# Nazukixv/LiteASR

Hardware: AMD Instinct MI355X
Metric: utterances/sec (U2-Conformer+CTC, 80-d fbank T≈1000) at 1/2/4/8 MI355X (higher is better)
Workload: dtype bf16; 1 GPU; U2-Conformer-small hybrid CTC-attention training step (fwd+loss+bwd+allreduce+clip+Noam/Adam); model=U2 enc 12x conformer d256 H4 ff2048, dec 6x, V 4233, global_batch=32, per_gpu_batch=32, seq_len=1000, label_len=40, parallelism=dp1, launch=hipgraph, ranks_seen=1, rank_launcher=env

## Files before the change

### include/liteasr_hip.h

```cpp
#ifndef LITEASR_HIP_H
#define LITEASR_HIP_H

#include <stdint.h>

#ifdef __cplusplus
extern "C" {
#endif

enum { LASR_F32 = 0, LASR_BF16 = 1, LASR_I32 = 2, LASR_I64 = 3, LASR_U8 = 4 };
enum { LASR_OK = 0, LASR_ERR_INVALID = -1, LASR_ERR_LAUNCH = -2 };
enum { LASR_ACT_NONE = 0, LASR_ACT_RELU = 1, LASR_ACT_SWISH = 2,
       LASR_ACT_GATE = 3 ,
       LASR_ACT_TANH = 4  };

const char* lasr_last_error(void);
int lasr_version(void);
int lasr_set_dropout_counter(const uint64_t* dev_counter);
int lasr_counter_add(uint64_t* dev_counter, uint64_t v, void* stream);

typedef struct lasr_gemm_args {
  int M, N, K;
  int batch, batch_div;
  const void* A; int64_t lda_m, lda_k, sa1, sa2;
  const void* B; int64_t ldb_n, ldb_k, sb1, sb2;
  void* C; int64_t ldc, sc1, sc2;
  int in_dtype;
  int c_dtype;
  float alpha; const float* alpha_dev;
  float beta;
  const float* bias;
  int act;
  void* zout;
  const void* aux; int aux_dtype; int64_t ldaux; int aux_act;
  float drop_p; uint64_t drop_seed;
  const void* res; int res_dtype; int64_t ldres; float res_scale;
  int split_k;
  void* workspace; int64_t workspace_bytes;
  float* rowsum;
  int zout_mode;
  int tile_m, tile_n;
  int ksub;
} lasr_gemm_args;
int lasr_gemm(const lasr_gemm_args* args, void* stream);
int lasr_gemm_ln_fwd(const lasr_gemm_args* args, const float* gamma, const float* beta, float eps, void* y,
                     int y_dtype, float* mean, float* rstd, void* stream);
int lasr_gemm_ln_bwd(const lasr_gemm_args* args, const void* x, int x_dtype, const float* gamma, const float* mean,
                     const float* rstd, const void* dres, int dres_dtype, void* dx, int dx_dtype, float* part,
                     int64_t part_floats, void* gb, int gb_dtype, float bscale, float bp, uint64_t bseed,
                     void* stream);
int lasr_gemm_qbias_bwd(const lasr_gemm_args* args, const void* dqu, const void* dqv, int dt, int B, int T, int H,
                        int dk, void* dqkv, int64_t ld, float* ws, int64_t ws_floats, void* stream);
float lasr_dropout_scale(float p);
#define LASR_PLAN_GLDS 1
#define LASR_PLAN_ROWSUM_FUSED 2
#define LASR_PLAN_KSUB2 4
#define LASR_PLAN_WIDE 8
int lasr_gemm_plan(const lasr_gemm_args* args, int* tile_m, int* tile_n, int* split_k, int* flags);

int lasr_gemm_dw_group(const lasr_gemm_args* args, int n, void* stream);
int lasr_gemm_dw_group_order(int longest_first);
int lasr_gemm_narrow_tiles(int on);

typedef struct lasr_reduce_seg {
  const float* part; int64_t N; int P; int accumulate;
  float* out0; float* out1; int64_t split;
} lasr_reduce_seg;
int lasr_reduce_multi(const lasr_reduce_seg* segs, int nseg, void* stream);

int lasr_colsum(const void* X, int dtype, int64_t M, int64_t N, int64_t ldx,
                float* out, int accumulate, float* workspace, int64_t ws_floats, void* stream);

int lasr_layernorm_fwd(const void* x, int x_dtype, int64_t rows, int D, const float* gamma,
                       const float* beta, float eps, void* y, int y_dtype, float* mean,
                       float* rstd, void* y2, int y2_dtype, float p2, uint64_t seed2,
                       void* stream);
int lasr_layernorm2_fwd(const float* x, int64_t rows, int D, const float* g1, const float* b1,
                        const float* g2, const float* b2, float eps, float* y, float* mean1,
                        float* rstd1, void* z, float* mean2, float* rstd2, void* stream);
int lasr_layernorm_bwd(const void* x, int x_dtype, const void* dy, int dy_dtype, int64_t rows,
                       int D, const float* gamma, const float* mean, const float* rstd,
                       const void* dres, int dres_dtype, void* dx, int dx_dtype,
                       float* dgamma, float* dbeta, float* workspace, int64_t ws_floats,
                       void* gb, int gb_dtype, float bscale, float bp, uint64_t bseed,
                       void* stream);
int lasr_layernorm2_bwd(const float* x1, const void* dy1, int dy1_dtype, const float* dres1, int64_t rows, int D,
                        const float* g1, const float* mean1, const float* rstd1, float* part1, const float* x2,
                        const float* g2, const float* mean2, const float* rstd2, float* dx2, float* part2, void* gb2,
                        int gb2_dtype, float bscale, float bp, uint64_t bseed, void* stream);
typedef struct lasr_row_ln_args {
  int M, D, K;
  const void* A; int64_t lda;
  const void* W; int64_t ldw;
  const float* gamma1; const float* beta1; float eps;
  float* mean1; float* rstd1;
  const float* bias; const float* res; float res_scale; float drop_p; uint64_t drop_seed;
  float* out; void* y1; int y1_dtype;
  const float* gamma2; const float* beta2; void* y2; float* mean2; float* rstd2;
  const float* x; const float* dres; float* dx; void* gb; float bscale; float bp; uint64_t bseed;
  float* part; float* dgamma; float* dbeta;
} lasr_row_ln_args;
int lasr_linear_res_ln(const lasr_row_ln_args* args, void* stream);
int lasr_linear_dx_ln_bwd(const lasr_row_ln_args* args, void* stream);

int lasr_branch_grad(const void* dx, int dx_dtype, int64_t n, void* gb, int gb_dtype,
                     float scale, float p, uint64_t seed, void* stream);

int lasr_ctc_fwd(const void* logits, int ldt, int B, int T, int V, int64_t ld, const int32_t* targets,
                 int Lmax, const int32_t* ilen, const int32_t* tlen, float* lse, float* lp,
                 float* alpha, float* beta, float* nll, void* stream);
int lasr_ctc_lattice(int B, int T, int Lmax, const int32_t* targets, const int32_t* ilen, const int32_t* tlen,
                     const float* lp, float* alpha, float* beta, float* nll, void* stream);
int lasr_ctc_bwd(const void* logits, int ldt, int B, int T, int V, int64_t ld, const int32_t* targets,
                 int Lmax, const int32_t* ilen, const int32_t* tlen, const float* lse,
                 const float* lp, const float* alpha, const float* nll, float* beta,
                 int beta_ready, void* grad, int gdt, float gscale, const float* gdev, void* stream);

int lasr_lsm_kl_fwd(const void* logits, int ldt, int R, int V, int64_t ld, const int32_t* target,
                    int ignore, float smoothing, float* lse, float* loss_rows, void* stream);
int lasr_lsm_kl_bwd(const void* logits, int ldt, int R, int V, int64_t ld, const int32_t* target,
                    int ignore, float smoothing, const float* lse, void* grad, int gdt,
                    float gscale, const float* gdev, void* stream);
int lasr_loss_combine(const float* a, int na, float wa, const float* b, int nb, float wb,
                      float* out, void* stream);

int lasr_qbias_fwd(const void* qkv, int dt, int B, int T, int H, int dk, int64_t ld_qkv,
                   const float* bias_u, const float* bias_v, void* qu, void* qv, void* stream);
int lasr_qbias_bwd(const void* dqu, const void* dqv, int dt, int B, int T, int H, int dk,
                   void* dqkv, int64_t ld_dqkv, float* dbias_u, float* dbias_v,
                   float* workspace, int64_t ws_floats, void* stream);
int lasr_attn_softmax_fwd(const float* s_ac, const float* s_bd, int relpos, int B, int H,
                          int Tq, int Tk, int ldS, const uint8_t* mask, int64_t mask_sb,
                          int64_t mask_sq, void* P, int pdt, float drop_p, uint64_t seed,
                          void* Praw, void* stream);
int lasr_attn_softmax_bwd(const void* P, int pdt, const float* dPd, int B, int H, int Tq, int Tk,
                          int ldS, const uint8_t* mask, int64_t mask_sb, int64_t mask_sq,
                          float drop_p, uint64_t seed, void* dS, int dsdt, void* stream);
int lasr_relshift_bwd(const void* dS, int dt, int Z, int T, int ldS, void* dBD, void* stream);
int lasr_relattn_fwd(const void* qu, const void* qv, int64_t ldq, const void* k, const void* v,
                     int64_t ldkv, const void* pos, int64_t ldp, int B, int H, int T, int dk,
                     const uint8_t* mask, int64_t mask_sb, int64_t mask_sq, float scale,
                     float* stats, void* ctx, int64_t ldc, void* stream);
int lasr_relattn_fwd_qb(const void* q, int64_t ldqin, const float* bu, const float* bv, void* qu, void* qv,
                        int64_t ldq, const void* k, const void* v, int64_t ldkv, const void* pos, int64_t ldp,
                        int B, int H, int T, int dk, const uint8_t* mask, int64_t mask_sb, int64_t mask_sq,
                        float scale, float* stats, void* ctx, int64_t ldc, void* stream);
int lasr_relattn_bwd(const void* qu, const void* qv, int64_t ldq, const void* k, const void* v,
                     int64_t ldkv, const void* pos, int64_t ldp, int B, int H, int T, int dk,
                     const uint8_t* mask, int64_t mask_sb, int64_t mask_sq, float scale,
                     const float* stats, const void* ctx, const void* dctx, int64_t ldc,
                     float* Dbuf, void* dqu, void* dbd, int ldS, int dbd_head_major, void* dk_out,
                     void* dv_out, int64_t lddkv, void* stream);
int lasr_attn_fwd(const void* q, int64_t ldq, const void* k, const void* v, int64_t ldkv, int B, int H,
                  int Tq, int Tk, int dk, const uint8_t* mask, int64_t mask_sb, int64_t mask_sq, float scale,
                  float* stats, void* ctx, int64_t ldc, void* stream);
int lasr_attn_bwd(const void* q, int64_t ldq, const void* k, const void* v, int64_t ldkv, int B, int H,
                  int Tq, int Tk, int dk, const uint8_t* mask, int64_t mask_sb, int64_t mask_sq, float scale,
                  const float* stats, const void* ctx, const void* dctx, int64_t ldc, float* Dbuf, void* dq,
                  void* dk_out, void* dv_out, int64_t lddkv, void* stream);
int lasr_attn_fwd_split(const void* q, int64_t ldq, const void* k, const void* v, int64_t ldkv, int B, int H,
                        int Tq, int Tk, int dk, const uint8_t* mask, int64_t mask_sb, int64_t mask_sq, float scale,
                        float* stats, void* ctx, int64_t ldc, int nsplit, float* work, int64_t work_floats,
                        void* stream);
int lasr_attn_bwd_split(const void* q, int64_t ldq, const void* k, const void* v, int64_t ldkv, int B, int H,
                        int Tq, int Tk, int dk, const uint8_t* mask, int64_t mask_sb, int64_t mask_sq, float scale,
                        const float* stats, const void* ctx, const void* dctx, int64_t ldc, float* Dbuf, void* dq,
                        void* dk_out, void* dv_out, int64_t lddkv, int nsplit, float* work, int64_t work_floats,
                        void* stream);
int64_t lasr_attn_split_work(int B, int H, int Tq, int dk, int nsplit);
int lasr_attn_split_count(int B, int H, int Tq, int Tk);
int lasr_reduce_batch(const float* src, int B, int H, int T, int dk, void* dst, int dt,
                      void* stream);

int lasr_conv1_fwd(const float* x, int B, int T, int F, int C, const float* w,
                   const float* bias, void* y1, int dt, void* stream);
int lasr_conv1_bwd(const float* x, int B, int T, int F, int C, const void* dy1, int dt,
                   float* dw, float* db, float* workspace, int64_t ws_floats, void* stream);
int lasr_im2col3x3s2(const void* y1, int dt, int B, int T1, int F1, int C, void* col,
                     void* stream);
int lasr_col2im3x3s2(const void* dcol, int dt, int B, int T1, int F1, int C,
                     const void* y1, void* dy1, void* stream);
#define LASR_CONV2_FWD 0
#define LASR_CONV2_DW 1
#define LASR_CONV2_DX 2
#define LASR_CONV2_DX_W1 3
typedef struct lasr_conv2_args {
  int mode;
  int B, T1, F1, C;
  const void* y1;
  const void* w2p;
  const float* bias;
  const void* dy2; int64_t dy2_rows;
  void* out;
  float* rowsum;
  void* workspace; int64_t workspace_bytes;
  const float* x; int T, F;
  float* dw1; float* db1;
} lasr_conv2_args;
int lasr_conv2_gemm(const lasr_conv2_args* args, void* stream);
int64_t lasr_conv2_dx_w1_workspace(int B, int T1, int F1, int C);
typedef struct lasr_cif_args {
  int B, T, D, U;
  const float* z; const int* plen; const int* ylen; const float* h;
  float* alpha; float* acc; uint8_t* fired; int* row; float* sum_alpha; float* mae; float* out;
  const float* gout; const float* gsum; float* dz; float* dh;
} lasr_cif_args;
int lasr_cif_fwd(const lasr_cif_args* args, void* stream);
int lasr_cif_bwd(const lasr_cif_args* args, void* stream);
typedef struct lasr_cif_infer_args {
  int B, T, D;
  const float* z; const int* plen; const float* h;
  float* alpha; float* acc; uint8_t* fired; int* row; float* sum_alpha; int* ulen; int* count; float* out;
} lasr_cif_infer_args;
int lasr_cif_infer(const lasr_cif_infer_args* args, void* stream);
int lasr_glancing_mix(int64_t rows, int D, const uint8_t* replace, const float* a, const float* b,
// ... 171 lines not shown
```

### liteasr_amd/_native.py

```python

from __future__ import annotations

import ctypes as C
import os

_HERE = os.path.dirname(os.path.abspath(__file__))
LIB_PATH = os.path.join(_HERE, "lib", "libliteasr_hip.so")

F32, BF16, I32, I64, U8 = 0, 1, 2, 3, 4
ACT_NONE, ACT_RELU, ACT_SWISH, ACT_GATE, ACT_TANH = 0, 1, 2, 3, 4

_p = C.c_void_p
_i = C.c_int
_l = C.c_int64
_f = C.c_float
_u = C.c_uint64


class GemmArgs(C.Structure):

    _fields_ = [
        ("M", _i), ("N", _i), ("K", _i),
        ("batch", _i), ("batch_div", _i),
        ("A", _p), ("lda_m", _l), ("lda_k", _l), ("sa1", _l), ("sa2", _l),
        ("B", _p), ("ldb_n", _l), ("ldb_k", _l), ("sb1", _l), ("sb2", _l),
        ("C", _p), ("ldc", _l), ("sc1", _l), ("sc2", _l),
        ("in_dtype", _i), ("c_dtype", _i),
        ("alpha", _f), ("alpha_dev", _p),
        ("beta", _f),
        ("bias", _p),
        ("act", _i),
        ("zout", _p),
        ("aux", _p), ("aux_dtype", _i), ("ldaux", _l), ("aux_act", _i),
        ("drop_p", _f), ("drop_seed", _u),
        ("res", _p), ("res_dtype", _i), ("ldres", _l), ("res_scale", _f),
        ("split_k", _i), ("workspace", _p), ("workspace_bytes", _l),
        ("rowsum", _p),
        ("zout_mode", _i),
        ("tile_m", _i), ("tile_n", _i), ("ksub", _i),
    ]


class Conv2Args(C.Structure):

    _fields_ = [
        ("mode", _i),
        ("B", _i), ("T1", _i), ("F1", _i), ("C", _i),
        ("y1", _p), ("w2p", _p), ("bias", _p),
        ("dy2", _p), ("dy2_rows", _l),
        ("out", _p), ("rowsum", _p),
        ("workspace", _p), ("workspace_bytes", _l),
        ("x", _p), ("T", _i), ("F", _i),
        ("dw1", _p), ("db1", _p),
    ]


CONV2_FWD, CONV2_DW, CONV2_DX, CONV2_DX_W1 = 0, 1, 2, 3


class CifArgs(C.Structure):

    _fields_ = [
        ("B", _i), ("T", _i), ("D", _i), ("U", _i),
        ("z", _p), ("plen", _p), ("ylen", _p), ("h", _p),
        ("alpha", _p), ("acc", _p), ("fired", _p), ("row", _p), ("sum_alpha", _p), ("mae", _p), ("out", _p),
        ("gout", _p), ("gsum", _p), ("dz", _p), ("dh", _p),
    ]


class CifInferArgs(C.Structure):

    _fields_ = [
        ("B", _i), ("T", _i), ("D", _i),
        ("z", _p), ("plen", _p), ("h", _p),
        ("alpha", _p), ("acc", _p), ("fired", _p), ("row", _p), ("sum_alpha", _p), ("ulen", _p), ("count", _p),
        ("out", _p),
    ]


class RowLnArgs(C.Structure):

    _fields_ = [
        ("M", _i), ("D", _i), ("K", _i),
        ("A", _p), ("lda", _l), ("W", _p), ("ldw", _l),
        ("gamma1", _p), ("beta1", _p), ("eps", _f), ("mean1", _p), ("rstd1", _p),
        ("bias", _p), ("res", _p), ("res_scale", _f), ("drop_p", _f), ("drop_seed", _u),
        ("out", _p), ("y1", _p), ("y1_dtype", _i),
        ("gamma2", _p), ("beta2", _p), ("y2", _p), ("mean2", _p), ("rstd2", _p),
        ("x", _p), ("dres", _p), ("dx", _p), ("gb", _p), ("bscale", _f), ("bp", _f), ("bseed", _u),
        ("part", _p), ("dgamma", _p), ("dbeta", _p),
    ]


class ReduceSeg(C.Structure):

    _fields_ = [("part", _p), ("N", _l), ("P", _i), ("accumulate", _i), ("out0", _p), ("out1", _p),
                ("split", _l)]


RNNT_SEARCH_MAX_LAYERS = 8


class RnntSearchArgs(C.Structure):

    _fields_ = [
        ("Tcap", _i), ("layers", _i), ("dec_dim", _i), ("H", _i), ("J", _i), ("V", _i),
        ("node_cap", _i), ("slot_cap", _i),
        ("w_dtype", _i),
        ("arena", _p), ("arena_bytes", _l),
        ("embed", _p),
        ("Wih", _p * RNNT_SEARCH_MAX_LAYERS), ("Whh", _p * RNNT_SEARCH_MAX_LAYERS),
        ("bih", _p * RNNT_SEARCH_MAX_LAYERS), ("bhh", _p * RNNT_SEARCH_MAX_LAYERS),
        ("Wd", _p), ("Wj", _p), ("bj", _p), ("enc_proj", _p),
    ]


SIGNATURES = {
    "lasr_version": [],
    "lasr_last_error": [],
    "lasr_set_dropout_counter": [_p],
    "lasr_counter_add": [_p, _u, _p],
    "lasr_gemm": [C.POINTER(GemmArgs), _p],
    "lasr_gemm_plan": [C.POINTER(GemmArgs), _p, _p, _p, _p],
    "lasr_gemm_dw_group": [C.POINTER(GemmArgs), _i, _p],
    "lasr_gemm_dw_group_order": [_i],
    "lasr_gemm_narrow_tiles": [_i],
    "lasr_relattn_fwd": [_p, _p, _l, _p, _p, _l, _p, _l, _i, _i, _i, _i, _p, _l, _l, _f, _p, _p, _l, _p],
    "lasr_relattn_fwd_qb": [_p, _l, _p, _p, _p, _p, _l, _p, _p, _l, _p, _l, _i, _i, _i, _i, _p, _l, _l, _f, _p, _p,
                            _l, _p],
    "lasr_attn_fwd": [_p, _l, _p, _p, _l, _i, _i, _i, _i, _i, _p, _l, _l, _f, _p, _p, _l, _p],
    "lasr_attn_bwd": [_p, _l, _p, _p, _l, _i, _i, _i, _i, _i, _p, _l, _l, _f, _p, _p, _p, _l, _p, _p, _p, _p,
                      _l, _p],
    "lasr_attn_fwd_split": [_p, _l, _p, _p, _l, _i, _i, _i, _i, _i, _p, _l, _l, _f, _p, _p, _l, _i, _p, _l, _p],
    "lasr_attn_bwd_split": [_p, _l, _p, _p, _l, _i, _i, _i, _i, _i, _p, _l, _l, _f, _p, _p, _p, _l, _p, _p, _p,
                            _p, _l, _i, _p, _l, _p],
    "lasr_attn_split_work": [_i, _i, _i, _i, _i],
    "lasr_attn_split_count": [_i, _i, _i, _i],
    "lasr_relattn_bwd": [_p, _p, _l, _p, _p, _l, _p, _l, _i, _i, _i, _i, _p, _l, _l, _f, _p, _p, _p, _l,
                         _p, _p, _p, _i, _i, _p, _p, _l, _p],
    "lasr_reduce_multi": [C.POINTER(ReduceSeg), _i, _p],
    "lasr_linear_res_ln": [C.POINTER(RowLnArgs), _p],
    "lasr_linear_dx_ln_bwd": [C.POINTER(RowLnArgs), _p],
    "lasr_dropout_scale": [_f],
    "lasr_colsum": [_p, _i, _l, _l, _l, _p, _i, _p, _l, _p],
    "lasr_layernorm2_fwd": [_p, _l, _i, _p, _p, _p, _p, _f, _p, _p, _p, _p, _p, _p, _p],
    "lasr_layernorm_fwd": [_p, _i, _l, _i, _p, _p, _f, _p, _i, _p, _p, _p, _i, _f, _u, _p],
    "lasr_layernorm_bwd": [_p, _i, _p, _i, _l, _i, _p, _p, _p, _p, _i, _p, _i, _p, _p, _p, _l,
                           _p, _i, _f, _f, _u, _p],
    "lasr_layernorm2_bwd": [_p, _p, _i, _p, _l, _i, _p, _p, _p, _p, _p, _p, _p, _p, _p, _p, _p, _i, _f, _f, _u,
                            _p],
    "lasr_branch_grad": [_p, _i, _l, _p, _i, _f, _f, _u, _p],
    "lasr_ctc_fwd": [_p, _i, _i, _i, _i, _l, _p, _i, _p, _p, _p, _p, _p, _p, _p, _p],
    "lasr_ctc_lattice": [_i, _i, _i, _p, _p, _p, _p, _p, _p, _p, _p],
    "lasr_rnnt_fwd": [_p, _i, _i, _i, _i, _i, _l, _p, _i, _p, _p, _i, _p, _p, _p, _p, _p, _p],
    "lasr_rnnt_bwd": [_p, _i, _i, _i, _i, _i, _l, _p, _i, _p, _p, _i, _p, _p, _p, _p, _p, _p, _i, _f, _p, _p],
    "lasr_joint_fwd": [_p, _p, _i, _i, _i, _i, _p, _i, _p],
    "lasr_joint_reduce": [_p, _i, _i, _i, _i, _i, _p, _p, _i, _p],
    "lasr_lstm_cell_fwd": [_p, _l, _p, _p, _i, _i, _p, _p, _i, _l, _p],
    "lasr_lstm_cell_bwd": [_p, _l, _p, _p, _p, _p, _i, _l, _p, _p, _i, _i, _p, _i, _l, _p, _p],
    "lasr_ctc_bwd": [_p, _i, _i, _i, _i, _l, _p, _i, _p, _p, _p, _p, _p, _p, _p, _i, _p, _i, _f, _p, _p],
    "lasr_lsm_kl_fwd": [_p, _i, _i, _i, _l, _p, _i, _f, _p, _p, _p],
    "lasr_lsm_kl_bwd": [_p, _i, _i, _i, _l, _p, _i, _f, _p, _p, _i, _f, _p, _p],
    "lasr_loss_combine": [_p, _i, _f, _p, _i, _f, _p, _p],
    "lasr_qbias_fwd": [_p, _i, _i, _i, _i, _i, _l, _p, _p, _p, _p, _p],
    "lasr_qbias_bwd": [_p, _p, _i, _i, _i, _i, _i, _p, _l, _p, _p, _p, _l, _p],
    "lasr_attn_softmax_fwd": [_p, _p, _i, _i, _i, _i, _i, _i, _p, _l, _l, _p, _i, _f, _u, _p, _p],
    "lasr_attn_softmax_bwd": [_p, _i, _p, _i, _i, _i, _i, _i, _p, _l, _l, _f, _u, _p, _i, _p],
    "lasr_relshift_bwd": [_p, _i, _i, _i, _i, _p, _p],
    "lasr_reduce_batch": [_p, _i, _i, _i, _i, _p, _i, _p],
    "lasr_conv1_fwd": [_p, _i, _i, _i, _i, _p, _p, _p, _i, _p],
    "lasr_conv1_bwd": [_p, _i, _i, _i, _i, _p, _i, _p, _p, _p, _l, _p],
    "lasr_conv2_gemm": [C.POINTER(Conv2Args), _p],
    "lasr_conv2_dx_w1_workspace": [_i, _i, _i, _i],
    "lasr_cif_fwd": [C.POINTER(CifArgs), _p],
    "lasr_cif_bwd": [C.POINTER(CifArgs), _p],
    "lasr_cif_infer": [C.POINTER(CifInferArgs), _p],
    "lasr_glancing_mix": [_l, _i, _p, _p, _p, _p, _p, _i, _p],
    "lasr_im2col3x3s2": [_p, _i, _i, _i, _i, _i, _p, _p],
    "lasr_col2im3x3s2": [_p, _i, _i, _i, _i, _i, _p, _p, _p],
    "lasr_permute_last2": [_p, _i, _l, _l, _l, _p, _i, _i, _i, _p],
    "lasr_glu_dwconv_fwd": [_p, _i, _i, _i, _i, _i, _p, _p, _p, _i, _p, _p],
    "lasr_dwconv_nparts": [_i, _i],
    "lasr_bn_finalize": [_p, _i, _i, _f, _f, _p, _p, _p, _p, _p, _p, _p, _p, _p, _i, _p],
    "lasr_bn_act_fwd": [_p, _i, _l, _i, _p, _p, _p, _i, _i, _p],
    "lasr_bn_act_bwd": [_p, _i, _p, _i, _l, _i, _p, _p, _p, _p, _p, _p, _p, _p, _i, _p, _l, _i, _i, _p],
    "lasr_glu_dwconv_bwd": [_p, _i, _p, _i, _i, _i, _i, _i, _p, _p, _p, _p, _p, _l, _p],
    "lasr_bn_act_glu_dwconv_bwd": [_p, _i, _p, _i, _i, _i, _i, _p, _p, _p, _p, _p, _p, _p, _p, _l, _i, _i,
                                   _p, _i, _i, _p, _p, _p, _p, _p, _l, _p],
    "lasr_cast": [_p, _i, _p, _i, _l, _p],
    "lasr_scale_add": [_p, _i, _p, _i, _f, _f, _p, _i, _l, _p],
    "lasr_embed_pe_fwd": [_p, _i, _i, _i, _p, _p, _f, _f, _u, _p, _i, _p],
    "lasr_embed_bwd": [_p, _i, _i, _p, _i, _f, _f, _u, _p, _p],
    "lasr_pe_fwd": [_p, _i, _l, _i, _i, _p, _f, _f, _u, _p, _i, _p],
    "lasr_u2_prep": [_p, _p, _p, _i, _i, _i, _i, _i, _i, _i, _p, _p, _p, _p, _p, _p, _p, _p],
    "lasr_u2_prep_ld": [_p, _p, _p, _i, _i, _i, _i, _i, _i, _i, _p, _p, _p, _p, _i, _p, _i, _p, _p, _p],
    "lasr_gemm_qbias_bwd": [C.POINTER(GemmArgs), _p, _p, _i, _i, _i, _i, _i, _p, _l, _p, _l, _p],
    "lasr_gemm_ln_fwd": [C.POINTER(GemmArgs), _p, _p, _f, _p, _i, _p, _p, _p],
    "lasr_gemm_ln_bwd": [C.POINTER(GemmArgs), _p, _i, _p, _p, _p, _p, _i, _p, _i, _p, _l, _p, _i, _f, _f, _u, _p],
    "lasr_u2_prep_chunk": [_p, _p, _p, _i, _i, _i, _i, _i, _i, _i, _p, _p, _u, _i,
                           _p, _p, _p, _p, _i, _p, _p, _i, _p, _p, _p],
    "lasr_pcm_to_float": [_p, _l, _p, _p],
    "lasr_fbank": [_p, _l, _i, _l, _p, _i, _p, _p, _i, _p, _p, _p, _i, _p],
    "lasr_resample_i16": [_p, _l, _i, _l, _p, _p, _i, _p, _l, _p, _l, _l, _p],
    "lasr_sumsq_nparts": [_l],
    "lasr_sumsq_partial": [_p, _l, _p, _l, _p],
    "lasr_adam_step": [_p, _p, _i, _p, _p, _p, _l, _p, _i, _p, _f, _i, _f, _f, _f, _f, _f, _f,
                       _f, _f, _p],
    "lasr_fill": [_p, _i, _l, _f, _p],
    "lasr_spec_augment": [_p, _p, _p, _p, _i, _i, _i, _i, _i, _p, _l, _p],
    "lasr_spec_augment_ws_bytes": [_i, _i],
    "lasr_logsoftmax_topk": [_p, _i, _l, _i, _l, _i, _p, _p, _p, _p, _p],
    "lasr_rnnt_search_workspace": [_i, _i, _i, _i, _i, _i, _i],
    "lasr_rnnt_search_init": [C.POINTER(RnntSearchArgs), _i, _p],
    "lasr_rnnt_search_expand": [C.POINTER(RnntSearchArgs), _i, _p],
    "lasr_rescore_workspace": [_i, _i],
    "lasr_rescore_search": [_p, _l, _i, _i, _i, _i, _i, _p, _p, _p, _p],
    "lasr_rescore_prep": [_p, _l, _i, _i, _i, _i, _p, _p, _i, _p, _p, _p],
    "lasr_rescore_pick": [_p, _l, _i, _i, _p, C.c_double, _p],
    "lasr_w2v_conv0_fwd": [_p, _i, _i, _i, _i, _i, _p, _p, _p, _p],
    "lasr_w2v_conv0_dw_parts": [_i, _i],
    "lasr_w2v_conv0_dw": [_p, _p, _i, _i, _i, _i, _i, _i, _p, _p, _l, _p],
    "lasr_w2v_ln_act_fwd": [_p, _i, _l, _i, _p, _p, _f, _i, _p, _i, _p, _p, _p],
    "lasr_w2v_ln_act_bwd": [_p, _i, _p, _i, _l, _i, _p, _p, _p, _p, _i, _p, _i, _p, _p, _p, _l, _p],
    "lasr_w2v_col2im1d": [_p, _i, _i, _i, _i, _i, _i, _i, _p, _p],
    "lasr_w2v_group_pack": [_p, _i, _i, _i, _i, _i, _i, _p, _i, _p, _p, _i, _p],
    "lasr_w2v_group_unpack": [_p, _i, _p, _i, _p, _i, _i, _i, _i, _p, _p],
    "lasr_w2v_group_colsum": [_p, _i, _i, _l, _i, _p, _p],
    "lasr_w2v_mask_fwd": [_p, _p, _i, _i, _i, _i, _p, _p],
    "lasr_w2v_mask_bwd": [_p, _p, _i, _i, _i, _i, _p, _p],
    "lasr_w2v_gather_rows": [_p, _i, _l, _l, _p, _i, _i, _i, _i, _p, _i, _p],
    "lasr_w2v_scatter_rows": [_p, _i, _p, _i, _i, _i, _i, _p, _l, _l, _i, _p],
    "lasr_w2v_gumbel_fwd": [_p, _i, _p, _u, _f, _i, _l, _i, _i, _p, _i, _p, _i, _p, _p],
    "lasr_w2v_gumbel_bwd": [_p, _i, _p, _u, _f, _i, _l, _i, _i, _p, _i, _p, _i, _p, _p, _i, _p, _p],
    "lasr_w2v_contrast_fwd": [_p, _p, _p, _p, _i, _i, _i, _i, _i, _f, _p, _p, _p, _p, _p],
    "lasr_w2v_contrast_bwd": [_p, _p, _p, _p, _i, _i, _i, _i, _i, _f, _p, _p, _p, _p, _p, _l, _p],
}
_RESTYPES = {"lasr_last_error": C.c_char_p, "lasr_spec_augment_ws_bytes": C.c_int64,
             "lasr_rnnt_search_workspace": C.c_int64, "lasr_rescore_workspace": C.c_int64,
             "lasr_conv2_dx_w1_workspace": C.c_int64, "lasr_attn_split_work": C.c_int64,
             "lasr_dropout_scale": C.c_float}


class NativeError(RuntimeError):
    pass


_lib = None


def load():
    global _lib
    if _lib is not None:
        return _lib
    want = os.environ.get("LITEASR_HIP_LIB")
    if want and os.path.abspath(want) != os.path.abspath(LIB_PATH):
        raise NativeError(f"LITEASR_HIP_LIB={want} does not select the library (this process loads {LIB_PATH}); "
                          "run `python tools/with_lib.py LIB script.py` to use another build")
    if not os.path.exists(LIB_PATH):
        raise NativeError(
            f"libliteasr_hip.so not found at {LIB_PATH}; build it with `make` "
            "(the HIP path has no fallback)"
        )
    lib = C.CDLL(LIB_PATH)
    for name, argtypes in SIGNATURES.items():
        fn = getattr(lib, name)
        fn.argtypes = argtypes
        fn.restype = _RESTYPES.get(name, C.c_int)
    _lib = lib
    return lib


def call(name, *args):
    lib = _lib if _lib is not None else load()
    rc = getattr(lib, name)(*args)
    if rc != 0:
        msg = lib.lasr_last_error().decode(errors="replace")
        raise NativeError(f"{name} failed ({rc}): {msg}")
    return rc


def exported_symbols():
    return sorted(SIGNATURES)
```

### liteasr_amd/csrc/gemm.hip

```cpp
#include "gemm_kernel.h"
#include <algorithm>


template <bool AKC, bool BKC, typename TC>
void launch_bf16(const GemmP& p, int BM, int BN, int ks, int nw, bool glds, dim3 grid, hipStream_t st);
#define LASR_EXTERN_LAUNCH(ak, bk)                                                                         \
  extern template void launch_bf16<ak, bk, float>(const GemmP&, int, int, int, int, bool, dim3, hipStream_t); \
  extern template void launch_bf16<ak, bk, bf16_t>(const GemmP&, int, int, int, int, bool, dim3, hipStream_t);
LASR_EXTERN_LAUNCH(true, true)
LASR_EXTERN_LAUNCH(true, false)
LASR_EXTERN_LAUNCH(false, true)
LASR_EXTERN_LAUNCH(false, false)
#undef LASR_EXTERN_LAUNCH

template <typename TC>
static void dispatch(const GemmP& p, bool akc, bool bkc, int bf16in, int BM, int BN, int ks, int nw, bool glds,
                     dim3 grid, hipStream_t st) {
  if (bf16in) {
    if (akc && bkc) launch_bf16<true, true, TC>(p, BM, BN, ks, nw, glds, grid, st);
    else if (akc) launch_bf16<true, false, TC>(p, BM, BN, ks, nw, glds, grid, st);
    else if (bkc) launch_bf16<false, true, TC>(p, BM, BN, ks, nw, glds, grid, st);
    else launch_bf16<false, false, TC>(p, BM, BN, ks, nw, glds, grid, st);
  } else {
    if (akc && bkc) gemm_f32_kernel<true, true, TC><<<grid, 256, 0, st>>>(p);
    else if (akc) gemm_f32_kernel<true, false, TC><<<grid, 256, 0, st>>>(p);
    else if (bkc) gemm_f32_kernel<false, true, TC><<<grid, 256, 0, st>>>(p);
    else gemm_f32_kernel<false, false, TC><<<grid, 256, 0, st>>>(p);
  }
}

static int narrow_n_tiles = 1;
extern "C" int lasr_gemm_narrow_tiles(int on) {
  narrow_n_tiles = on != 0;
  return LASR_OK;
}

static void gemm_plan(const lasr_gemm_args* a, int* BMo, int* BNo, int* splito, int* kso = nullptr,
                      int* nwo = nullptr) {
  int nw = 4;
  const int batch = a->batch > 0 ? a->batch : 1;
  const bool bf = a->in_dtype == LASR_BF16;
  int BM = 64, BN = 64;
  int split = a->split_k > 0 ? a->split_k : 1;
  const bool plain = !a->act && !a->zout && !a->aux && !a->res && a->drop_p <= 0.f;
  const bool autosplit = a->split_k <= 0 && !a->zout && a->workspace;
  const int kt = (int)cdiv(a->K, 32);
  if (bf && autosplit && kt >= 16) {
    const bool very_long = kt >= 2048;
    BM = BN = 64;
    if (very_long) {
      BM = a->M >= 96 ? 128 : 64;
      BN = a->N >= 96 ? 128 : 64;
    } else if ((int64_t)a->M * a->N > 768 * 256) {
      BM = a->M >= a->N ? 64 : 128;
      BN = a->M >= a->N ? 128 : 64;
    }
    const int64_t nb = cdiv(a->M, BM) * cdiv(a->N, BN) * (int64_t)batch;
    const int64_t target = a->lda_k == 1 ? 128 : (very_long || !plain ? 256 : 512);
    while (nb * split < target && split * 2 <= 64 && kt / (split * 2) >= 8) split *= 2;
  } else if (bf) {
    const int cfg[4][2] = {{128, 128}, {128, 64}, {64, 128}, {64, 64}};
    const int c0 = a->N <= 64 && narrow_n_tiles ? 3 : 0;
    for (int c = c0; c < 4; ++c) {
      const int64_t nb = cdiv(a->M, cfg[c][0]) * cdiv(a->N, cfg[c][1]) * (int64_t)batch;
      BM = cfg[c][0]; BN = cfg[c][1];
      if (nb >= 480) break;
    }
    if (BM == 128 && BN == 128 && a->N >= 256 && a->K >= 1024 && cdiv(a->M, 128) * batch >= 1024) BN = 256;
    if (BM == 128 && BN == 128 && (a->zout || a->aux || (a->act && a->drop_p > 0.f)) && a->N >= 1024) BN = 256;
  }
  if (!bf && autosplit) {
    const int64_t nb = cdiv(a->M, BM) * cdiv(a->N, BN) * (int64_t)batch;
    while (nb * split < 512 && split * 2 <= 32 && kt / (split * 2) >= 4) split *= 2;
  }
  if (bf && a->tile_m) {
    BM = a->tile_m;
    BN = a->tile_n;
    nw = 4;
  }
  if (a->split_k <= -2 && plain && a->workspace) split = -a->split_k;
  const int64_t rs_floats = a->rowsum ? (int64_t)split * a->M : 0;
  if (split > 1 && ((!plain && !autosplit && (a->split_k < 2 || a->zout)) || !a->workspace ||
                    a->workspace_bytes < ((int64_t)split * batch * a->M * a->N + rs_floats) * 4))
    split = 1;
  if (kso) {
    const int64_t kc = split > 1 ? cdiv(a->K, split) : a->K;
    const bool small = BM * BN <= 64 * 128;
    *kso = (bf && BM < 256 && BN < 256 && ((BM == 64 && BN == 64) || kc >= 1024 || (kc >= 512 && small))) ? 2 : 1;
    if (nw == 8) *kso = 2;
    else if (a->ksub) *kso = a->ksub;
  }
  if (nwo) *nwo = nw;
  *BMo = BM;
  *BNo = BN;
  *splito = split;
}

static bool gemm_uses_glds(const lasr_gemm_args* a) {
  if (a->in_dtype != LASR_BF16) return false;
  const bool akc = (a->lda_k == 1), bkc = (a->ldb_k == 1);
  const int64_t s_a = akc ? a->lda_m : a->lda_k;
  const int64_t s_b = bkc ? a->ldb_n : a->ldb_k;
  const bool a_vec = aligned16(a->A) && s_a % 8 == 0 && a->sa1 % 8 == 0 && a->sa2 % 8 == 0;
  const bool b_vec = aligned16(a->B) && s_b % 8 == 0 && a->sb1 % 8 == 0 && a->sb2 % 8 == 0;
  const int64_t M8 = cdiv(a->M, 8) * 8, N8 = cdiv(a->N, 8) * 8;
  return a_vec && b_vec && (akc || a->lda_k >= M8) && (bkc || a->ldb_k >= N8);
}

static bool tile_ok(int tm, int tn) {
  return (tm == 0 && tn == 0) || ((tm == 64 || tm == 128 || tm == 256) && (tn == 64 || tn == 128 || tn == 256) &&
                                  (tm < 256 || tn >= 128) && (tn < 256 || tm >= 128));
}

extern "C" int lasr_gemm_plan(const lasr_gemm_args* a, int* tile_m, int* tile_n, int* split_k, int* flags) {
  LASR_CHECK_ARG(a && tile_m && tile_n && split_k, "lasr_gemm_plan: null argument");
  int ks = 1, nw = 4;
  gemm_plan(a, tile_m, tile_n, split_k, &ks, &nw);
  const bool glds = gemm_uses_glds(a);
  if (!glds) {
    *tile_m = std::min(*tile_m, 128);
    *tile_n = std::min(*tile_n, 128);
    nw = 4;
  }
  if (flags) {
    *flags = (glds ? LASR_PLAN_GLDS : 0) | (a->rowsum && glds && a->lda_k != 1 ? LASR_PLAN_ROWSUM_FUSED : 0) |
             (glds && ks == 2 && (*tile_m < 256 || nw == 8) ? LASR_PLAN_KSUB2 : 0) |
             (glds && nw == 8 ? LASR_PLAN_WIDE : 0);
  }
  return LASR_OK;
}

extern "C" int lasr_gemm(const lasr_gemm_args* a, void* stream) { return gemm_run(a, stream, nullptr); }

int gemm_run(const lasr_gemm_args* a, void* stream, GemmRowPost* post) {
  LASR_CHECK_ARG(a != nullptr, "lasr_gemm: null args");
  LASR_CHECK_ARG(a->M >= 0 && a->N >= 0 && a->K >= 0, "lasr_gemm: negative size");
  LASR_CHECK_ARG(a->in_dtype == LASR_F32 || a->in_dtype == LASR_BF16, "lasr_gemm: bad in_dtype");
  LASR_CHECK_ARG(a->c_dtype == LASR_F32 || a->c_dtype == LASR_BF16, "lasr_gemm: bad c_dtype");
  LASR_CHECK_ARG(a->lda_m == 1 || a->lda_k == 1, "lasr_gemm: A needs a unit stride");
  LASR_CHECK_ARG(a->ldb_n == 1 || a->ldb_k == 1, "lasr_gemm: B needs a unit stride");
  LASR_CHECK_ARG(a->A && a->B && a->C, "lasr_gemm: null operand");
  LASR_CHECK_ARG(a->zout_mode == 0 || a->zout_mode == 1, "lasr_gemm: zout_mode must be 0 or 1");
  LASR_CHECK_ARG(a->act != LASR_ACT_GATE && (!a->aux || a->aux_act != LASR_ACT_NONE),
                 "lasr_gemm: act GATE is only an aux_act; aux needs an aux_act");
  LASR_CHECK_ARG(tile_ok(a->tile_m, a->tile_n) && a->ksub >= 0 && a->ksub <= 2,
                 "lasr_gemm: tile override must be 64/128/256 x 64/128/256 (256 only beside >= 128) or 0 x 0, "
                 "ksub 0, 1 or 2");
  if (a->M == 0 || a->N == 0 || a->batch == 0) return LASR_OK;
  const int batch = a->batch > 0 ? a->batch : 1;
  const int bdiv = a->batch_div > 0 ? a->batch_div : 1;
  LASR_CHECK_ARG(batch == 1 || (!a->aux && !a->res && !a->zout && !a->rowsum),
                 "lasr_gemm: aux/res/zout/rowsum only supported for batch == 1");
  LASR_CHECK_ARG(!a->rowsum || a->lda_m == 1, "lasr_gemm: rowsum needs an M-contiguous A");

  GemmP p;
  p.M = a->M; p.N = a->N; p.K = a->K; p.batch = batch; p.batch_div = bdiv;
  p.A = a->A; p.lda_m = a->lda_m; p.lda_k = a->lda_k; p.sa1 = a->sa1; p.sa2 = a->sa2;
  p.B = a->B; p.ldb_n = a->ldb_n; p.ldb_k = a->ldb_k; p.sb1 = a->sb1; p.sb2 = a->sb2;
  p.C = a->C; p.ldc = a->ldc; p.sc1 = a->sc1; p.sc2 = a->sc2;
  p.alpha = a->alpha; p.alpha_dev = a->alpha_dev; p.beta = a->beta;
  p.bias = a->bias; p.act = a->act; p.zout = a->zout; p.zout_mode = a->zout_mode;
  p.aux = a->aux; p.aux_dtype = a->aux_dtype; p.ldaux = a->ldaux; p.aux_act = a->aux_act;
  p.drop = mkdrop(a->drop_p, a->drop_seed);
  p.res = a->res; p.res_dtype = a->res_dtype; p.ldres = a->ldres; p.res_scale = a->res_scale;

  const bool akc = (a->lda_k == 1);
  const bool bkc = (a->ldb_k == 1);
  const bool bf = a->in_dtype == LASR_BF16;
  {
    const int64_t s_a = akc ? a->lda_m : a->lda_k;
    const int64_t s_b = bkc ? a->ldb_n : a->ldb_k;
    p.a_vec = bf && aligned16(a->A) && s_a % 8 == 0 && a->sa1 % 8 == 0 && a->sa2 % 8 == 0;
    p.b_vec = bf && aligned16(a->B) && s_b % 8 == 0 && a->sb1 % 8 == 0 && a->sb2 % 8 == 0;
  }
  p.c_vec = aligned16(a->C) && a->ldc % 8 == 0 && a->sc1 % 8 == 0 && a->sc2 % 8 == 0 &&
            (!a->zout || aligned16(a->zout));
  p.aux_vec = a->aux && aligned16(a->aux) && a->ldaux % 8 == 0;
  p.res_vec = a->res && aligned16(a->res) && a->ldres % 8 == 0;
  p.ws_vec = a->N % 8 == 0;
  p.bias_vec = a->bias && aligned16(a->bias);
  {
    auto al4 = [](const void* q, int dtp) {
      return ((uintptr_t)q & (dtp == LASR_F32 ? 15 : 7)) == 0;
    };
    const int cdt = a->c_dtype;
    p.v4 = a->N % 4 == 0 && a->ldc % 4 == 0 && a->sc1 % 4 == 0 && a->sc2 % 4 == 0 && al4(a->C, cdt) &&
           (!a->zout || al4(a->zout, cdt)) && (!a->bias || aligned16(a->bias)) &&
           (!a->aux || (a->ldaux % 4 == 0 && al4(a->aux, a->aux_dtype))) &&
           (!a->res || (a->ldres % 4 == 0 && al4(a->res, a->res_dtype))) &&
           (!a->workspace || aligned16(a->workspace));
  }
  {
    const int nsrc = (a->aux ? 1 : 0) + (a->res ? 1 : 0);
    const bool base_ok = p.c_vec && a->beta == 0.f;
    const bool src_ok = nsrc == 1 && a->N % 8 == 0 && (a->aux ? p.aux_vec : p.res_vec);
    p.epi_mode = !base_ok ? 2 : nsrc == 0 ? 0 : src_ok ? 1 : 2;
  }

  int BM, BN, split, ks, nw;
  gemm_plan(a, &BM, &BN, &split, &ks, &nw);
  p.split_k = split;
  const int kstep = bf ? 32 : 16;
  p.kchunk = split > 1 ? (int)(cdiv(cdiv(a->K, split), kstep) * kstep) : a->K;
  p.ws = (float*)a->workspace;
  p.rowsum = nullptr;
  p.rs_ws = nullptr;

  hipStream_t st = (hipStream_t)stream;
  const bool glds = gemm_uses_glds(a);
  if (!glds) {
    BM = std::min(BM, 128);
    BN = std::min(BN, 128);
    nw = 4;
  }
  dim3 grid((unsigned)cdiv(a->N, BN), (unsigned)cdiv(a->M, BM), (unsigned)(batch * split));
  LASR_CHECK_ARG(grid.y <= 65535 && grid.z <= 65535, "lasr_gemm: grid too large");
  const bool rs_fused = a->rowsum && glds && !akc;
  if (rs_fused) {
    p.rowsum = a->rowsum;
    if (split > 1) p.rs_ws = p.ws + (int64_t)split * batch * a->M * a->N;
  }
  if (a->c_dtype == LASR_F32) dispatch<float>(p, akc, bkc, bf, BM, BN, ks, nw, glds, grid, st);
  else dispatch<bf16_t>(p, akc, bkc, bf, BM, BN, ks, nw, glds, grid, st);
  int rc = lasr_check_launch("lasr_gemm");
  if (!rc && split > 1 && a->split_k >= 0 && post) {
    const int r = post->launch(p, post->ctx, st);
    if (r < 0) return r;
    post->done = r;
    if (r) {
      rc = lasr_check_launch("lasr_gemm/splitk_reduce_post");
      if (rc || !a->rowsum || rs_fused) return rc;
    }
  }
  if (!rc && split > 1 && a->split_k >= 0 && !(post && post->done)) {
    const int64_t total = (int64_t)a->M * a->N * batch;
    const int nblk = (int)std::min<int64_t>(cdiv(p.v4 ? total / 4 : total, 256), 4096);
    if (a->c_dtype == LASR_F32) splitk_reduce_kernel<float><<<nblk, 256, 0, st>>>(p);
    else splitk_reduce_kernel<bf16_t><<<nblk, 256, 0, st>>>(p);
    rc = lasr_check_launch("lasr_gemm/splitk_reduce");
  }
  if (rc || !a->rowsum || rs_fused) return rc;
  const int64_t used = split > 1 ? (int64_t)split * batch * a->M * a->N : 0;
  LASR_CHECK_ARG(a->workspace && a->workspace_bytes / 4 > used, "lasr_gemm: no workspace left for the rowsum");
  return lasr_colsum(a->A, a->in_dtype, a->K, a->M, a->lda_k, a->rowsum, 1, (float*)a->workspace + used,
                     a->workspace_bytes / 4 - used, stream);
}


int launch_dw_group(const DwGroupP& g, int BM, int BN, int blocks, bool serial, hipStream_t st);
static int dw_group_lpt = 1;
extern "C" int lasr_gemm_dw_group_order(int longest_first) {
  dw_group_lpt = longest_first != 0;
  return LASR_OK;
}

extern "C" int lasr_gemm_dw_group(const lasr_gemm_args* args, int n, void* stream) {
  LASR_CHECK_ARG(args && n >= 1 && n <= LASR_DW_GROUP_MAX, "lasr_gemm_dw_group: 1..%d problems", LASR_DW_GROUP_MAX);
  DwGroupP g = {};
  g.n = n;
  int ord[LASR_DW_GROUP_MAX];
  int64_t work[LASR_DW_GROUP_MAX];
  auto planned = [](const lasr_gemm_args* a) {
    lasr_gemm_args b = *a;
    if (b.split_k <= -2 && !b.workspace) {
      b.workspace = (void*)(uintptr_t)16;
      b.workspace_bytes = INT64_MAX;
    }
    return b;
  };
  for (int i = 0; i < n; ++i) {
    const lasr_gemm_args pa = planned(args + i), *a = &pa;
    int bm, bn, sp, ks;
    gemm_plan(a, &bm, &bn, &sp, &ks);
    work[i] = a->split_k == 1 || sp <= 1 ? a->K : cdiv(a->K, sp);
    ord[i] = i;
  }
  if (dw_group_lpt && !(args[0].split_k <= -2 && !args[0].workspace))
    std::stable_sort(ord, ord + n, [&](int x, int y) { return work[x] > work[y]; });
  int BM0 = 0, BN0 = 0, blocks = 0;
  bool all_serial = false;
  for (int i = 0; i < n; ++i) {
    const bool serial = args[ord[i]].split_k <= -2 && !args[ord[i]].workspace;
    const lasr_gemm_args pa = planned(args + ord[i]), *a = &pa;
    LASR_CHECK_ARG(a->in_dtype == LASR_BF16 && a->c_dtype == LASR_F32, "lasr_gemm_dw_group: bf16 in, fp32 partials");
    LASR_CHECK_ARG(a->lda_m == 1 && a->lda_k != 1 && a->ldb_n == 1 && a->ldb_k != 1,
                   "lasr_gemm_dw_group: A M-contiguous and B N-contiguous (dW = dY^T X)");
    const bool direct = a->split_k == 1;
    LASR_CHECK_ARG((direct || (a->split_k < 0 && a->workspace)) && (a->batch <= 1) && a->M > 0 && a->N > 0 &&
                       a->K > 0,
                   "lasr_gemm_dw_group: partials-only problems with a workspace, or direct (split_k 1) ones");
    LASR_CHECK_ARG(!serial || (a->C && a->ldc >= a->N && (a->beta == 0.f || a->beta == 1.f) && a->alpha == 1.f &&
                               !a->alpha_dev && a->split_k >= -64),
                   "lasr_gemm_dw_group: a serial problem needs C, ldc >= N, beta 0 or 1, alpha 1, <= 64 slices");
    LASR_CHECK_ARG(i == 0 || serial == all_serial, "lasr_gemm_dw_group: serial and slab problems mixed");
    all_serial = serial;
    LASR_CHECK_ARG(!direct || (a->C && a->ldc >= a->N && (a->beta == 0.f || a->beta == 1.f) && a->alpha == 1.f &&
                               !a->alpha_dev),
                   "lasr_gemm_dw_group: a direct problem needs C, ldc >= N, beta 0 or 1, alpha 1");
    LASR_CHECK_ARG(i == 0 || direct == (g.direct[0] != 0), "lasr_gemm_dw_group: direct and split problems mixed");
    LASR_CHECK_ARG(!a->act && !a->zout && !a->aux && !a->res && a->drop_p <= 0.f && !a->bias,
                   "lasr_gemm_dw_group: no epilogue");
    LASR_CHECK_ARG(gemm_uses_glds(a), "lasr_gemm_dw_group: operands not LDS-DMA eligible");
    int BM, BN, split, ks;
    gemm_plan(a, &BM, &BN, &split, &ks);
    if (direct) split = 2;
    LASR_CHECK_ARG(split > 1, "lasr_gemm_dw_group: plan is not a split-K launch");
    if (((BM == 128 && BN == 64) || (BM == 64 && BN == 128)) && a->M >= 128 && a->N >= 128) {
      BM = BN = 128;
      if (a->M >= 256 && a->N >= 256 && !direct) {
        BM = 256;
        BN = 128;
      }
    }
    LASR_CHECK_ARG(i == 0 || (BM == BM0 && BN == BN0), "lasr_gemm_dw_group: problems plan different tiles");
    BM0 = BM;
    BN0 = BN;
    if (direct) split = 1;
    g.M[i] = a->M; g.N[i] = a->N; g.K[i] = a->K;
    g.split[i] = split;
    g.kchunk[i] = direct ? a->K : (int)(cdiv(cdiv(a->K, split), 32) * 32);
    g.direct[i] = direct;
    g.C[i] = (float*)a->C; g.ldc[i] = a->ldc; g.beta[i] = a->beta; g.rowsum[i] = a->rowsum;
    g.v4[i] = serial ? a->N % 4 == 0 && aligned16(a->C) && a->ldc % 4 == 0
                     : a->N % 4 == 0 && aligned16(direct ? a->C : a->workspace);
    g.A[i] = a->A; g.lda[i] = a->lda_k;
    g.B[i] = a->B; g.ldb[i] = a->ldb_k;
    g.ws[i] = serial ? nullptr : (float*)a->workspace;
    g.rs_ws[i] = a->rowsum && !direct && !serial ? (float*)a->workspace + (int64_t)split * a->M * a->N : nullptr;
    g.start[i] = blocks;
    const int64_t nb = cdiv(a->M, BM) * cdiv(a->N, BN) * (int64_t)(serial ? 1 : split);
    LASR_CHECK_ARG(blocks + nb + 8 < (1ll << 31), "lasr_gemm_dw_group: too many blocks");
    blocks += (int)cdiv(nb, 8) * 8;
  }
  g.start[n] = blocks;
  static const int slice_xcd = [] { const char* e = getenv("LASR_DW_SLICE_XCD"); return e && e[0] ? atoi(e) : 1; }();
  g.slice_xcd = slice_xcd;
  LASR_CHECK_ARG(launch_dw_group(g, BM0, BN0, blocks, all_serial, (hipStream_t)stream) == 0,
                 "lasr_gemm_dw_group: no grouped instance for tile %dx%d", BM0, BN0);
  return lasr_check_launch("lasr_gemm_dw_group");
}
```

Measured before the change: 3514 utterances/sec.

## Add phased software-pipelined GEMM kernel for single-wave large-K shapes

Adds a specialized 128x64 bf16 GEMM kernel with a 6-stage global-to-LDS ring buffer. It interleaves MFMA issue with LDS fragment reads and DMA issue under scheduling barriers and raised wave priority. The path is used by default (mode 1) only for GEMMs with K>=1024 whose tile count falls between 3/4 and 1x the CU count, with plain bf16 or residual-dropout f32 epilogues. The aim is to hide memory latency on occupancy-1, single-wave GEMMs such as the FF2048 down-projection. It adds a launch counter and a mode switch. The risk is lower throughput than the existing tuned kernels on the shapes it takes over.

```diff
diff --git a/include/liteasr_hip.h b/include/liteasr_hip.h
--- a/include/liteasr_hip.h
+++ b/include/liteasr_hip.h
@@ -60,6 +60,8 @@
 int lasr_gemm_dw_group(const lasr_gemm_args* args, int n, void* stream);
 int lasr_gemm_dw_group_order(int longest_first);
 int lasr_gemm_narrow_tiles(int on);
+int lasr_gemm_phased(int mode);
+long long lasr_gemm_phased_launches(void);
 
 typedef struct lasr_reduce_seg {
   const float* part; int64_t N; int P; int accumulate;
diff --git a/liteasr_amd/_native.py b/liteasr_amd/_native.py
--- a/liteasr_amd/_native.py
+++ b/liteasr_amd/_native.py
@@ -125,6 +125,8 @@
     "lasr_gemm_dw_group": [C.POINTER(GemmArgs), _i, _p],
     "lasr_gemm_dw_group_order": [_i],
     "lasr_gemm_narrow_tiles": [_i],
+    "lasr_gemm_phased": [_i],
+    "lasr_gemm_phased_launches": [],
     "lasr_relattn_fwd": [_p, _p, _l, _p, _p, _l, _p, _l, _i, _i, _i, _i, _p, _l, _l, _f, _p, _p, _l, _p],
     "lasr_relattn_fwd_qb": [_p, _l, _p, _p, _p, _p, _l, _p, _p, _l, _p, _l, _i, _i, _i, _i, _p, _l, _l, _f, _p, _p,
                             _l, _p],
@@ -238,7 +240,7 @@
 _RESTYPES = {"lasr_last_error": C.c_char_p, "lasr_spec_augment_ws_bytes": C.c_int64,
              "lasr_rnnt_search_workspace": C.c_int64, "lasr_rescore_workspace": C.c_int64,
              "lasr_conv2_dx_w1_workspace": C.c_int64, "lasr_attn_split_work": C.c_int64,
-             "lasr_dropout_scale": C.c_float}
+             "lasr_dropout_scale": C.c_float, "lasr_gemm_phased_launches": C.c_int64}
 
 
 class NativeError(RuntimeError):
diff --git a/liteasr_amd/csrc/gemm.hip b/liteasr_amd/csrc/gemm.hip
--- a/liteasr_amd/csrc/gemm.hip
+++ b/liteasr_amd/csrc/gemm.hip
@@ -1,4 +1,5 @@
 #include "gemm_kernel.h"
+#include "gemm_phase.h"
 #include <algorithm>
 
 
@@ -220,9 +221,12 @@
     p.rowsum = a->rowsum;
     if (split > 1) p.rs_ws = p.ws + (int64_t)split * batch * a->M * a->N;
   }
-  if (a->c_dtype == LASR_F32) dispatch<float>(p, akc, bkc, bf, BM, BN, ks, nw, glds, grid, st);
+  const bool phased = gemm_phased_launch(a, p, glds, st);
+  if (phased) {
+  } else if (a->c_dtype == LASR_F32) dispatch<float>(p, akc, bkc, bf, BM, BN, ks, nw, glds, grid, st);
   else dispatch<bf16_t>(p, akc, bkc, bf, BM, BN, ks, nw, glds, grid, st);
   int rc = lasr_check_launch("lasr_gemm");
+  if (phased && !rc) gemm_phased_count();
   if (!rc && split > 1 && a->split_k >= 0 && post) {
     const int r = post->launch(p, post->ctx, st);
     if (r < 0) return r;
diff --git a/liteasr_amd/csrc/gemm_phase.h b/liteasr_amd/csrc/gemm_phase.h
--- /dev/null
+++ b/liteasr_amd/csrc/gemm_phase.h
@@ -0,0 +1,5 @@
+#pragma once
+#include "gemm_kernel.h"
+
+bool gemm_phased_launch(const lasr_gemm_args* a, const GemmP& p, bool glds, hipStream_t st);
+void gemm_phased_count();
diff --git a/liteasr_amd/csrc/gemm_phase.hip b/liteasr_amd/csrc/gemm_phase.hip
--- /dev/null
+++ b/liteasr_amd/csrc/gemm_phase.hip
@@ -0,0 +1,255 @@
+#include "gemm_phase.h"
+
+#include <atomic>
+#include <type_traits>
+
+namespace {
+
+constexpr int PH_BM = 128, PH_BN = 64;
+
+template <int GL, int NMAX>
+LASR_DEV void wait_stages(int n) {
+  if constexpr (NMAX > 0) {
+    if (n >= NMAX) { wait_vmcnt<GL * NMAX>(); return; }
+    wait_stages<GL, NMAX - 1>(n);
+  } else {
+    wait_vmcnt<0>();
+  }
+}
+
+LASR_DEV v4i ds_b128_at(uint32_t addr, int off) {
+  v4i r;
+  asm volatile("ds_read_b128 %0, %1 offset:%2" : "=v"(r) : "v"(addr), "n"(off));
+  return r;
+}
+LASR_DEV v2i ds_tr_at(uint32_t addr) {
+  v2i r;
+  asm volatile("ds_read_b64_tr_b16 %0, %1" : "=v"(r) : "v"(addr));
+  return r;
+}
+
+template <bool BKC>
+struct PhaseFrags {
+  v4i a[4];
+  v4i bk[BKC ? 2 : 1];
+  v2i bt[BKC ? 1 : 4];
+};
+
+template <bool BKC>
+LASR_DEV void frags_wait(PhaseFrags<BKC>& f) {
+  if constexpr (BKC)
+    asm volatile("s_waitcnt lgkmcnt(0)"
+                 : "+v"(f.a[0]), "+v"(f.a[1]), "+v"(f.a[2]), "+v"(f.a[3]), "+v"(f.bk[0]), "+v"(f.bk[1]));
+  else
+    asm volatile("s_waitcnt lgkmcnt(0)"
+                 : "+v"(f.a[0]), "+v"(f.a[1]), "+v"(f.a[2]), "+v"(f.a[3]), "+v"(f.bt[0]), "+v"(f.bt[1]),
+                   "+v"(f.bt[2]), "+v"(f.bt[3]));
+}
+
+LASR_DEV void pin() { __builtin_amdgcn_sched_barrier(0); }
+
+template <bool BKC, typename TC, int EPI, int S>
+__global__ __launch_bounds__(256, 1) void gemm_phase_kernel(GemmP p) {
+  constexpr int BM = PH_BM, BN = PH_BN, BK = 32, NT = 256;
+  constexpr int WM = 64, WN = 32, FM = 4, FN = 2;
+  constexpr int TILE = (BM + BN) * BK;
+  constexpr int STAGE = 2 * TILE, D = S - 1, GL = 2 * (BM + BN) * 4 / NT;
+  constexpr int MAIN_BYTES = S * STAGE * 2, EPI_BYTES = WM * (BN + 4) * 4;
+  static_assert(S >= 5, "vmcnt(GL * (D - 3)) must leave a stage in flight");
+  static_assert(MAIN_BYTES >= EPI_BYTES && MAIN_BYTES <= 160 * 1024, "ring size");
+  static_assert(GL * (D - 3) < 64, "vmcnt range");
+  __shared__ __attribute__((aligned(16))) char smem_epi[MAIN_BYTES];
+  bf16_t* smem = reinterpret_cast<bf16_t*>(smem_epi);
+  const int tid = threadIdx.x, lane = tid & 63, wid = tid >> 6;
+  const int wr = wid >> 1, wc = wid & 1;
+
+  const int nx = gridDim.x, ny = gridDim.y;
+  const int wg = xcd_remap(blockIdx.y * nx + blockIdx.x, nx * ny);
+  const int tx = wg % nx, ty = wg / nx;
+  const int m0 = ty * BM, n0 = tx * BN;
+  const int nst = p.K / (2 * BK);
+
+  f32x4 acc[FM][FN];
+#pragma unroll
+  for (int i = 0; i < FM; ++i)
+#pragma unroll
+    for (int j = 0; j < FN; ++j) acc[i][j] = (f32x4){0.f, 0.f, 0.f, 0.f};
+
+  uint32_t va[2], vb;
+#pragma unroll
+  for (int i = 0; i < 2; ++i) {
+    const int P = i * NT + tid, r = P >> 2, c = (P & 3) ^ swz(r);
+    va[i] = 2u * ((uint32_t)min(m0 + r, p.M - 1) * (uint32_t)p.lda_m + (uint32_t)c * 8u);
+  }
+  if constexpr (BKC) {
+    const int r = tid >> 2, c = (tid & 3) ^ swz(r);
+    vb = 2u * ((uint32_t)min(n0 + r, p.N - 1) * (uint32_t)p.ldb_n + (uint32_t)c * 8u);
+  } else {
+    constexpr int CPR = BN / 8;
+    const int k = tid / CPR, ps = tid % CPR;
+    const int ls = ((((ps >> 1) ^ htr<BN>(k))) << 1) | (ps & 1);
+    const int gc = min(n0 + ls * 8, ((p.N + 7) & ~7) - 8);
+    vb = 2u * ((uint32_t)k * (uint32_t)p.ldb_k + (uint32_t)gc);
+  }
+  const char* adma = (const char*)p.A;
+  const char* bdma = (const char*)p.B;
+  const int64_t bstep = BKC ? 2 * BK : 2 * BK * p.ldb_k;
+  const int wid_s = __builtin_amdgcn_readfirstlane(wid);
+  auto issue_sub = [&](int slot, int u) {
+    if (LASR_EXP & 4) return;
+    bf16_t* dst = smem + slot * STAGE + u * TILE + wid_s * 512;
+    __builtin_amdgcn_global_load_lds((gptr_t)(adma + va[0]), (lptr_t)dst, 16, 0, 0);
+    __builtin_amdgcn_global_load_lds((gptr_t)(adma + va[1]), (lptr_t)(dst + NT * 8), 16, 0, 0);
+    __builtin_amdgcn_global_load_lds((gptr_t)(bdma + vb), (lptr_t)(dst + BM * BK), 16, 0, 0);
+  };
+  auto advance = [&]() {
+    adma += 2 * BK;
+    bdma += bstep;
+  };
+
+  const uint32_t lds0 = (uint32_t)(uintptr_t)(lptr_t)smem;
+  const uint32_t a_off = lds0 + 2u * (uint32_t)lds_off(wr * WM + (lane & 15), lane >> 4);
+  [[maybe_unused]] const uint32_t bk_off =
+      lds0 + 2u * (uint32_t)(BM * BK + lds_off(wc * WN + (lane & 15), lane >> 4));
+  [[maybe_unused]] uint32_t bt_off[FN][2];
+  if constexpr (!BKC)
+#pragma unroll
+    for (int j = 0; j < FN; ++j) {
+      frag_tr_offsets<BN>(wc * WN + j * 16, lane, bt_off[j]);
+      bt_off[j][0] += lds0 + 2u * BM * BK;
+      bt_off[j][1] += lds0 + 2u * BM * BK;
+    }
+  auto read_part = [&](PhaseFrags<BKC>& f, uint32_t sub, int n) {
+    if (n == 0) {
+      f.a[0] = ds_b128_at(a_off + sub, 0);
+      f.a[1] = ds_b128_at(a_off + sub, 1024);
+    } else if (n == 1) {
+      f.a[2] = ds_b128_at(a_off + sub, 2048);
+      f.a[3] = ds_b128_at(a_off + sub, 3072);
+    } else if constexpr (BKC) {
+      f.bk[0] = ds_b128_at(bk_off + sub, 0);
+      f.bk[1] = ds_b128_at(bk_off + sub, 1024);
+    } else {
+      f.bt[0] = ds_tr_at(bt_off[0][0] + sub);
+      f.bt[1] = ds_tr_at(bt_off[0][1] + sub);
+      f.bt[2] = ds_tr_at(bt_off[1][0] + sub);
+      f.bt[3] = ds_tr_at(bt_off[1][1] + sub);
+    }
+  };
+  auto mfma = [&](const PhaseFrags<BKC>& f, int n) {
+    const int i = n >> 1, j = n & 1;
+    const bf16x8 af = __builtin_bit_cast(bf16x8, f.a[i]);
+    bf16x8 bfr;
+    if constexpr (BKC) bfr = __builtin_bit_cast(bf16x8, f.bk[j]);
+    else bfr = frag_from_raw(f.bt + 2 * j);
+    if (LASR_EXP & 1) {
+      acc[i][j][0] += (float)af[0] + (float)bfr[0];
+      return;
+    }
+    acc[i][j] = __builtin_amdgcn_mfma_f32_16x16x32_bf16(bfr, af, acc[i][j], 0, 0, 0);
+  };
+  auto group = [&](const PhaseFrags<BKC>& cur, PhaseFrags<BKC>& nxt, uint32_t nsub, bool dma, int slot, int u) {
+    __builtin_amdgcn_s_setprio(1);
+#pragma unroll
+    for (int n = 0; n < 8; ++n) {
+      mfma(cur, n);
+      pin();
+      if (n < 3) read_part(nxt, nsub, n);
+      pin();
+    }
+    if (dma) issue_sub(slot, u);
+    advance();
+    pin();
+    __builtin_amdgcn_s_setprio(0);
+  };
+
+  PhaseFrags<BKC> f0, f1;
+#pragma unroll
+  for (int t = 0; t < D; ++t)
+    if (t < nst) {
+      issue_sub(t, 0);
+      advance();
+      issue_sub(t, 1);
+      advance();
+    }
+  wait_stages<GL, D - 2>(min(D, nst) - 2);
+  __builtin_amdgcn_s_barrier();
+#pragma unroll
+  for (int n = 0; n < 3; ++n) read_part(f0, 0u, n);
+  int slot = 0;
+  for (int kt = 0; kt < nst; ++kt) {
+    const bool dma = kt + D < nst;
+    if (kt + D <= nst) wait_vmcnt<GL * (D - 3)>();
+    else wait_stages<GL, D - 3>(nst - 1 - (kt + 2));
+    __builtin_amdgcn_s_barrier();
+    const int nslot = slot + 1 == S ? 0 : slot + 1;
+    const int dslot = slot == 0 ? S - 1 : slot - 1;
+    const uint32_t sub0 = (uint32_t)slot * (STAGE * 2);
+    frags_wait<BKC>(f0);
+    group(f0, f1, sub0 + TILE * 2, dma, dslot, 0);
+    frags_wait<BKC>(f1);
+    group(f1, f0, (uint32_t)nslot * (STAGE * 2), dma, dslot, 1);
+    slot = nslot;
+  }
+  asm volatile("s_waitcnt lgkmcnt(0)" ::: "memory");
+  __syncthreads();
+  __builtin_assume(p.split_k <= 1 && p.epi_mode < 2);
+  gemm_epilogue<BM, BN, TC, true, G_LIN, 4, EPI>(p, acc, smem_epi, m0, n0, 0, 0, 0, 0);
+}
+
+constexpr int PH_S = 6;
+
+template <bool BKC>
+void launch_phase(const GemmP& p, int epi, dim3 grid, hipStream_t st) {
+  if (epi == EPI_RES_DROP) gemm_phase_kernel<BKC, float, EPI_RES_DROP, PH_S><<<grid, 256, 0, st>>>(p);
+  else gemm_phase_kernel<BKC, bf16_t, EPI_PLAIN, PH_S><<<grid, 256, 0, st>>>(p);
+}
+
+std::atomic<long long> phased_launches{0};
+std::atomic<int> phased_mode{1};
+
+int cu_count() {
+  static const int n = [] {
+    int dev = 0, v = 0;
+    if (hipGetDevice(&dev) != hipSuccess) return 0;
+    if (hipDeviceGetAttribute(&v, hipDeviceAttributeMultiprocessorCount, dev) != hipSuccess) return 0;
+    return v;
+  }();
+  return n;
+}
+
+}
+
+bool gemm_phased_launch(const lasr_gemm_args* a, const GemmP& p, bool glds, hipStream_t st) {
+  const int mode = phased_mode.load(std::memory_order_relaxed);
+  if (!mode) return false;
+  if (!glds || a->lda_k != 1 || p.batch != 1 || p.split_k > 1 || a->rowsum || a->zout) return false;
+  if (a->K < 64 || a->K % 64 != 0) return false;
+  const int e = epi_code(p);
+  const bool res_drop = e == EPI_RES_DROP && a->c_dtype == LASR_F32;
+  const bool plain = e == EPI_PLAIN && a->c_dtype == LASR_BF16;
+  if (!res_drop && !plain) return false;
+  const bool bkc = a->ldb_k == 1;
+  const int64_t a_bytes = 2 * (int64_t)a->M * a->lda_m, b_bytes = 2 * (bkc ? (int64_t)a->N * a->ldb_n : 32 * a->ldb_k);
+  if (a_bytes >= (1ll << 32) || b_bytes >= (1ll << 32)) return false;
+  const int64_t tiles = cdiv(a->M, PH_BM) * cdiv(a->N, PH_BN);
+  if (mode != 2) {
+    const int cus = cu_count();
+    if (a->K < 1024 || cus <= 0 || tiles > cus || tiles * 4 < (int64_t)cus * 3) return false;
+  }
+  if (cdiv(a->M, PH_BM) > 65535) return false;
+  dim3 grid((unsigned)cdiv(a->N, PH_BN), (unsigned)cdiv(a->M, PH_BM), 1);
+  if (bkc) launch_phase<true>(p, e, grid, st);
+  else launch_phase<false>(p, e, grid, st);
+  return true;
+}
+
+void gemm_phased_count() { phased_launches.fetch_add(1, std::memory_order_relaxed); }
+
+extern "C" int lasr_gemm_phased(int mode) {
+  LASR_CHECK_ARG(mode >= 0 && mode <= 2, "lasr_gemm_phased: mode 0 (never), 1 (by size) or 2 (force)");
+  phased_mode.store(mode, std::memory_order_relaxed);
+  return LASR_OK;
+}
+
+extern "C" long long lasr_gemm_phased_launches(void) { return phased_launches.load(std::memory_order_relaxed); }
```

After: 3555 utterances/sec (median of 6 runs). +1.2%, better.
